# alex-petrenko/sample-factory

Hardware: NVIDIA H100
Metric: env-steps/sec (sampler+learner) at 4096 envs (higher is better)
Workload: dtype f32 (3-pass tf32 hi/lo operand split on wgmma, fp32 accumulate)

## Files before the change

sample_factory_b200/csrc/gemm_tc.cu:

```cuda
#include <cuda.h>

#include <cstdlib>
#include <cudaTypedefs.h>

#include "common.cuh"
#include "gemm.h"
#include "heads_tail.cuh"
#include "tc_ptx.cuh"
#include "wgmma_tile.cuh"

namespace sfb {

constexpr int kProducerRegs = 40;
constexpr int kConsumerRegs = 232;

template <bool A_MN, bool B_MN, bool SPLIT3, bool HEADS, bool F16, bool RES, bool DW16>
__device__ __forceinline__ void gemm_tc_body(const CUtensorMap& tmap_a, const CUtensorMap& tmap_b, float* __restrict__ C,
                                             int64_t ldc, int64_t M, int N, int K, int k_chunk, int splits,
                                             const TcEpilogue& epi, const float* __restrict__ a_bound,
                                             const float* __restrict__ b_bound, unsigned long long* __restrict__ trace) {
    static_assert(!F16 || (!A_MN && SPLIT3), "fp16-split engine: K-major activations, 3-pass");
    static_assert(!DW16 || (A_MN && B_MN && SPLIT3 && !HEADS && !F16 && !RES), "fp16 dW form: MN-major operands, plain epilogue");
    if (trace && threadIdx.x == 0) trace[blockIdx.x * kTraceWords + 8] = tc_now();
    using S = TcSmem<F16, DW16>;
    constexpr int KBK = S::KBK;
    constexpr int SA = S::A_STAGES, SB = S::B_STAGES;
    extern __shared__ uint8_t smem_raw[];
    uint8_t* smem = smem_align_1024(smem_raw);
    uint8_t* conv = smem + S::CONV_OFF;
    uint64_t* bars = reinterpret_cast<uint64_t*>(smem + S::BARS_OFF);
    uint64_t* full_a = bars;
    uint64_t* empty_a = bars + SA;
    uint64_t* full_b = bars + 2 * SA;
    uint64_t* empty_b = bars + 2 * SA + SB;
    int* s_last = reinterpret_cast<int*>(bars + 2 * (SA + SB));

    const int warp = threadIdx.x >> 5, lane = threadIdx.x & 31;
    const int tiles_n = (N + TBN - 1) / TBN;
    const int tiles_per_z = tiles_n * (int)((M + TBM - 1) / TBM);
    const int items = tiles_per_z * splits;

    if (threadIdx.x == 0) {
        asm volatile("prefetch.tensormap [%0];" ::"l"(&tmap_a) : "memory");
        asm volatile("prefetch.tensormap [%0];" ::"l"(&tmap_b) : "memory");
        for (int s = 0; s < SA; ++s) {
            mbar_init(&full_a[s], 1);
            mbar_init(&empty_a[s], 256);
// ... 29 lines not shown
                } else if (DW16) {
                    for (int b = 0; b < TBM / 32; ++b) tma_load_2d(pa + b * 4096, &tmap_a, &full_a[sa], (int)tc.m0 + 32 * b, k0);
                } else if (A_MN) {
                    tma_load_2d(pa, &tmap_a, &full_a[sa], (int)tc.m0, k0);
                } else {
                    tma_load_2d(pa, &tmap_a, &full_a[sa], k0, (int)tc.m0);
                }
                mbar_wait(&empty_b[sb], ((g / SB) & 1) ^ 1);
                mbar_expect_tx(&full_b[sb], S::B_SLOT);
                uint8_t* pb = smem + S::B_RING + sb * S::B_SLOT;
                if (F16) tma_load_3d(pb, &tmap_b, &full_b[sb], k0, tc.n0, 0);
                else if (B_MN) tma_load_2d(pb, &tmap_b, &full_b[sb], tc.n0, k0);
                else tma_load_2d(pb, &tmap_b, &full_b[sb], k0, tc.n0);
            }
            if (trace) trace[item * kTraceWords + 7] = tc_now();
            g0 += tc.num_kb;
        }
        return;
    }

    setmaxnreg_inc<kConsumerRegs>();
    const int ct = threadIdx.x - 128;
    const int wg = ct >> 7;

    const int a_shift = (F16 || DW16) ? f16_shift_for_bound(a_bound[0]) : 0;
    const float a_scale = pow2f_int(a_shift);
    const int b_shift = DW16 ? f16_shift_for_bound(b_bound[0]) : kF16WShift;
    const float b_scale = pow2f_int(b_shift);
    auto split_stage = [&](int g) {
        const int sa = g % SA, sb = g % SB;
        const uint8_t* pa = smem + sa * S::A_RAW;
        uint8_t* cv = conv + (g & 1) * S::CONV;
        mbar_wait(&full_a[sa], (g / SA) & 1);
        split_tile<A_MN, SPLIT3>(pa, cv, cv + S::A_HALF, ct);
        mbar_wait(&full_b[sb], (g / SB) & 1);
        split_tile<B_MN, SPLIT3>(smem + S::B_RING + sb * S::B_SLOT, cv + 2 * S::A_HALF, cv + 2 * S::A_HALF + S::B_HALF, ct);
        mbar_arrive(&empty_b[sb]);
        mbar_arrive(&empty_a[sa]);
        fence_proxy_async_smem();
    };
    constexpr int KS = KBK / 32;
    using Frags = F16Frags<KS>;
    auto load_frags = [&](int g, int h, Frags& f) {
        const int sa = g % SA;
        const uint8_t* pa = smem + sa * S::A_RAW;
        if (h == 0) mbar_wait(&full_a[sa], (g / SA) & 1);
// ... 94 lines not shown
                        wgmma_m64n128k8_tf32(cross, da_hi + o, db_lo + o, 1);
                        wgmma_m64n128k8_tf32(cross, da_lo + o, db_hi + o, 1);
                    }
                }
                wgmma_commit();
                if (kb + 1 < tc.num_kb) split_stage(g + 1);
                wgmma_wait_all();
                consumer_sync();
            }
        }
        g0 += tc.num_kb;
        if (tr) tr[4] = tc_now();
        if (F16 || DW16) {
            const float out_scale = pow2f_int(-(a_shift + b_shift));
#pragma unroll
            for (int i = 0; i < 64; ++i) acc[i] = __fmul_rn(fmaf(cross[i], 1.f / 2048.f, acc[i]), out_scale);
        } else if (SPLIT3) {
#pragma unroll
            for (int i = 0; i < 64; ++i) acc[i] += cross[i];
        }
        if (tr) tr[10] = tc_now_after(acc[63]);

        const int64_t row_base = tc.m0 + wg * 64 + ((ct >> 5) & 3) * 16 + (lane >> 2);
        if constexpr (HEADS) {
            switch (epi.act) {
                case SFB200_ACT_ELU: heads_tile<SFB200_ACT_ELU>(acc, tc, row_base, lane, C, ldc, M, N, epi, tr); break;
                case SFB200_ACT_RELU: heads_tile<SFB200_ACT_RELU>(acc, tc, row_base, lane, C, ldc, M, N, epi, tr); break;
                case SFB200_ACT_TANH: heads_tile<SFB200_ACT_TANH>(acc, tc, row_base, lane, C, ldc, M, N, epi, tr); break;
                default: heads_tile<SFB200_ACT_NONE>(acc, tc, row_base, lane, C, ldc, M, N, epi, tr); break;
            }
            if (epi.fin_counters) {
                const int mb = (int)(tc.m0 / TBM);
                __threadfence();
                consumer_sync();
                if (ct == 0) *s_last = (atomicAdd(&epi.fin_counters[mb], 1) == tiles_n - 1) ? 1 : 0;
                consumer_sync();
                if (*s_last) {
                    __threadfence();
                    const float pv = epi.fin.pv_scalar ? *epi.fin.pv_scalar : 0.f;
                    const uint64_t offset = epi.fin.offset_host + (epi.fin.offset_dev ? (uint64_t)*epi.fin.offset_dev : 0ull);
                    for (int r = ct >> 5; r < TBM; r += 8) {
                        const int64_t row = tc.m0 + r;
                        if (row < M) heads_finish_row(epi.head_part, 2 * tiles_n, M, row, lane, epi.fin, pv, offset);
                    }
                    if (ct == 0) epi.fin_counters[mb] = 0;
                }
            }
        } else if constexpr (RES) {
            if (tile_is_whole(tc, TBM, C, ldc, M, N, epi.aux, epi.ld_aux))
                store_tile_whole<3, SFB200_ACT_NONE>(acc, tc, row_base, lane, C, ldc, epi, tr);
            else
                store_tile_residual(acc, tc, row_base, lane, C, ldc, M, N, epi);
        } else {
// ... 95 lines not shown
        v = (e && e[0] == '1') ? 1 : 0;
    }
    return v == 1;
}

static thread_local unsigned long long* g_gemm_trace = nullptr;
static thread_local int64_t g_gemm_trace_words = 0;

static bool operand_ok(const float* p, int64_t ld) {
    return ((reinterpret_cast<uintptr_t>(p) & 15u) == 0) && (ld % 4 == 0) && ld > 0;
}

template <bool A_MN, bool B_MN, bool SPLIT3, bool HEADS, bool F16, bool RES, bool DW16>
static auto tc_kernel() {
    if constexpr (DW16) return gemm_dw_f16_kernel;
    else return gemm_wgmma_kernel<A_MN, B_MN, SPLIT3, HEADS, F16, RES>;
}

template <bool A_MN, bool B_MN, bool SPLIT3, bool HEADS = false, bool F16 = false, bool RES = false, bool DW16 = false>
static int launch_tc(const CUtensorMap& ta, const CUtensorMap& tb, float* C, int64_t ldc, int64_t M, int N, int K,
                     int k_chunk, int splits, const TcEpilogue& epi, cudaStream_t st, const float* a_bound = nullptr,
                     const float* b_bound = nullptr) {
    auto kern = tc_kernel<A_MN, B_MN, SPLIT3, HEADS, F16, RES, DW16>();
    constexpr int smem = TcSmem<F16, DW16>::TOTAL;
    static int ctas_per_sm = 0;
    if (!ctas_per_sm) {
        SFB_CUDA_OK(cudaFuncSetAttribute(kern, cudaFuncAttributeMaxDynamicSharedMemorySize, smem));
        SFB_CUDA_OK(cudaOccupancyMaxActiveBlocksPerMultiprocessor(&ctas_per_sm, kern, TC_THREADS, (size_t)smem));
        SFB_CHECK_ARG(ctas_per_sm > 0, "gemm_wgmma_kernel does not fit on this device");
    }
    const int64_t items = ceil_div(N, TBN) * ceil_div(M, TBM) * splits;
    const int64_t resident = (int64_t)ctas_per_sm * sm_count();
    SFB_CHECK_ARG(!g_gemm_trace || items * kTraceWords <= g_gemm_trace_words,
                  "gemm trace buffer too small: %lld work items need %lld words", (long long)items,
                  (long long)(items * kTraceWords));
    const dim3 grid((unsigned)(items < resident ? items : resident));
    if constexpr (DW16)
        SFB_CUDA_OK(launch_pdl(kern, grid, dim3(TC_THREADS), (size_t)smem, st, ta, tb, C, ldc, M, N, K, k_chunk, splits, epi,
                               a_bound, g_gemm_trace, b_bound));
    else
        SFB_CUDA_OK(launch_pdl(kern, grid, dim3(TC_THREADS), (size_t)smem, st, ta, tb, C, ldc, M, N, K, k_chunk, splits, epi,
                               a_bound, g_gemm_trace));
    SFB_LAUNCH_OK();
    return 0;
}

static int split_k_chunk(int K, int* splits) {
// ... 154 lines not shown
```

sample_factory_b200/csrc/rollout_fused.cu:

```cuda
#include <cuda.h>

#include <cstdlib>

#include "common.cuh"
#include "gemm.h"
#include "heads_tail.cuh"
#include "step_tail.cuh"
#include "tc_ptx.cuh"
#include "wgmma_tile.cuh"

namespace sfb {

constexpr int RF_THREADS = 384;
constexpr int RF_HEAD_AP = 9;
constexpr int RF_MAX_DIM = 128;
constexpr int RF_TRACE_WORDS = 32;
constexpr int RF_PRODUCER_REGS = 40;
constexpr int RF_CONSUMER_REGS = 232;

__host__ __device__ __forceinline__ bool rf_wide(int H2) { return H2 >= 256; }
__host__ __device__ __forceinline__ int rf_bm(int H2) { return rf_wide(H2) ? 64 : 128; }
__host__ __device__ __forceinline__ int rf_bn(int H2) { return rf_wide(H2) ? 256 : 128; }

template <bool F16>
struct RfSmem {
    static constexpr int STAGES = 2;
    static constexpr int KBK = F16 ? 64 : TBK;
    __host__ __device__ static constexpr int slot(int bm, int bn) { return F16 ? (bm + bn) * 256 : (bm + 3 * bn) * 128; }
    __host__ __device__ static constexpr int a_bytes(int bm) { return bm * KBK * 4; }
    __host__ __device__ static constexpr int b_hi(int bm, int bn) { return F16 ? bm * 256 : (bm + bn) * 128; }
    __host__ __device__ static constexpr int stage_tx(int bm, int bn) { return (bm + bn) * KBK * 4; }
    static constexpr int OFF_CONV_END = STAGES * slot(64, 256) + 64 * 256;
    static constexpr int OFF_PART = OFF_CONV_END + (F16 ? 64 * 256 : 0);
    static constexpr int OFF_B1 = OFF_PART + (F16 ? 256 * kHeadPartPad * 4 : 0);
    static constexpr int OFF_B2 = OFF_B1 + (F16 ? 256 * 4 : 0);
    static constexpr int OFF_HW = OFF_B2 + (F16 ? 256 * 4 : 0);
    static constexpr int OFF_HB = OFF_HW + (F16 ? RF_HEAD_AP * 256 * 4 : 0);
    static constexpr int OFF_BARS = OFF_HB + (F16 ? 16 * 4 : 0);
    static constexpr int OFF_CSTAT = OFF_BARS + 64;
    static constexpr int TOTAL = OFF_CSTAT + 2 * RF_MAX_DIM * 4 + 1024 ;
    static_assert(2 * STAGES * 8 <= 64 && TOTAL + 64 <= 227 * 1024, "shared memory");
    static_assert(STAGES * slot(128, 128) + 128 * 256 <= OFF_PART, "the 128 x 128 layout fits below the partials");
    static_assert(a_bytes(64) % 1024 == 0 && slot(64, 256) % 1024 == 0 && OFF_CONV_END % 1024 == 0,
                  "h1 staging boxes (slot A regions, conversion buffer, the buffer after it) on 1024 B swizzle atoms");
};


struct RolloutArgs {
    int64_t N; int T, K1, H1, H2;
    const float* b1; const float* b2; const float* wv; const float* wa; int A; const float* bv; const float* ba;
    float* h1; float* part; float* x_norm;
    float* values; int64_t values_rs; float* logits; int64_t logits_rs; float* actions; int64_t actions_rs;
    int32_t* env_actions; float* log_prob; int64_t lp_rs; float* pv_out; int64_t pv_rs; const float* pv_scalar;
    const float* noise; uint64_t seed; int64_t* sampler_step;
    const float* tape; int64_t tape_len; int64_t env_off; int term_period, trunc_period; int64_t* env_step;
    float* env_obs; float* env_rew; uint8_t* env_term; uint8_t* env_trunc;
    EpisodeArgs e;
    float* traj_obs; int64_t traj_obs_rs; const float* rnn; int rnn_dim; float* traj_rnn; int64_t traj_rnn_rs;
    ObsNorm n;
    unsigned long long* trace;
    const float* bound_x; const float* bound_h1;
};

__device__ __forceinline__ void cluster_arrive() { asm volatile("barrier.cluster.arrive.release.aligned;" ::: "memory"); }
__device__ __forceinline__ void cluster_wait() { asm volatile("barrier.cluster.wait.acquire.aligned;" ::: "memory"); }
__device__ __forceinline__ void cluster_sync_all() {
    cluster_arrive();
    cluster_wait();
}
__device__ __forceinline__ void fence_proxy_async_all() { asm volatile("fence.proxy.async.global;" ::: "memory"); }
__device__ __forceinline__ unsigned long long rf_now() {
    unsigned long long t;
    asm volatile("mov.u64 %0, %%globaltimer;" : "=l"(t));
    return t;
}
__device__ __forceinline__ uint32_t smid() {
    uint32_t r;
    asm volatile("mov.u32 %0, %%smid;" : "=r"(r));
    return r;
}
__device__ __forceinline__ uint32_t mapa_shared(uint32_t addr, uint32_t rank) {
    uint32_t r;
    asm volatile("mapa.shared::cluster.u32 %0, %1, %2;" : "=r"(r) : "r"(addr), "r"(rank));
    return r;
}
__device__ __forceinline__ void st_cluster_f4(uint32_t addr, float4 v) {
    asm volatile("st.shared::cluster.v4.f32 [%0], {%1, %2, %3, %4};" ::"r"(addr), "f"(v.x), "f"(v.y), "f"(v.z), "f"(v.w)
                 : "memory");
}
__device__ __forceinline__ uint32_t cluster_ctarank() {
    uint32_t r;
    asm volatile("mov.u32 %0, %%cluster_ctarank;" : "=r"(r));
    return r;
}

template <bool F16>
__device__ __forceinline__ void rf_produce(const CUtensorMap* tmap_x, const CUtensorMap* tmap_w1, const CUtensorMap* tmap_h1,
                                           const CUtensorMap* tmap_w2, int T, int K1, int H1, int bm, int bn, int m0, int n0,
                                           uint8_t* smem, uint64_t* full, uint64_t* empty, bool leader) {
    using S = RfSmem<F16>;
    constexpr int KBK = S::KBK;
    const int slot_bytes = S::slot(bm, bn), b_off = S::a_bytes(bm);
    const uint32_t stage_tx = (uint32_t)S::stage_tx(bm, bn);
    const int n1 = K1 / KBK, n2 = H1 / KBK;
    uint32_t pu = 0;
    auto weight = [&](const CUtensorMap* tb, int kb) {
        const uint32_t s = pu % S::STAGES;
        mbar_wait(&empty[s], ((pu / S::STAGES) & 1) ^ 1);
        mbar_expect_tx(&full[s], stage_tx);
        uint8_t* dst = smem + s * slot_bytes + b_off;
        if (F16) tma_load_3d(dst, tb, &full[s], 64 * kb, n0, 0);
// ... 140 lines not shown
#pragma unroll
        for (int jj = 0; jj < 16; ++jj) {
            const int j = 16 * h + jj;
            const int r = rt + 8 * (j & 1), c = (j >> 1) & 7;
            const float v0 = act_fwd_fast(acc[2 * j] + b[j & ~1], act);
            const float v1 = act_fwd_fast(acc[2 * j + 1] + b[j | 1], act);
            uint32_t hv, lv;
            f16_split2(v0 * scale, v1 * scale, hv, lv);
            uint8_t* dst = box[h] + r * 128 + (((c ^ r) & 7) << 4) + 4 * (lane & 3);
            *reinterpret_cast<uint32_t*>(dst) = hv;
            *reinterpret_cast<uint32_t*>(dst + plane_bytes) = lv;
        }
        fence_proxy_async_smem();
        consumer_sync();
        if (issuer) {
            tma_store_3d(tmap_h1, box[h], n0 + 64 * h, m0, 0);
            bulk_commit();
        }
    }
}

template <int ACT>
__device__ __forceinline__ void rf_heads_tile(float (&acc)[64], int nl, int p0, int rb, int lane, const float* b2,
                                              const float* hw, int A, uint32_t part, int rpc) {
    constexpr int JP = 16;
    const int nq = nl + 2 * (lane & 3);
    float b[32];
#pragma unroll
    for (int c = 0; c < 16; ++c) {
        b[2 * c] = b2[nq + 8 * c];
        b[2 * c + 1] = b2[nq + 8 * c + 1];
    }
#pragma unroll
    for (int j = 0; j < 32; ++j) {
        acc[2 * j] = act_fwd_ct<ACT>(acc[2 * j] + b[j & ~1]);
        acc[2 * j + 1] = act_fwd_ct<ACT>(acc[2 * j + 1] + b[j | 1]);
    }
#pragma unroll
    for (int half = 0; half < 2; ++half) {
        float hp[2][kHeadAP];
#pragma unroll
        for (int a = 0; a < kHeadAP; ++a) {
            float s[2] = {0.f, 0.f};
            if (a <= A) {
                const float* w = hw + a * 256 + nq + 64 * half;
                float2 wv[JP / 2];
#pragma unroll
                for (int jj = 0; jj < JP / 2; ++jj) wv[jj] = *reinterpret_cast<const float2*>(w + 8 * jj);
#pragma unroll
                for (int jj = 0; jj < JP / 2; ++jj) {
#pragma unroll
                    for (int rs = 0; rs < 2; ++rs) {
                        const int j = JP * half + 2 * jj + rs;
                        s[rs] = fmaf(acc[2 * j], wv[jj].x, s[rs]);
                        s[rs] = fmaf(acc[2 * j + 1], wv[jj].y, s[rs]);
                    }
                }
            }
#pragma unroll
            for (int rs = 0; rs < 2; ++rs) {
                s[rs] += __shfl_xor_sync(0xffffffffu, s[rs], 1);
                s[rs] += __shfl_xor_sync(0xffffffffu, s[rs], 2);
                hp[rs][a] = s[rs];
            }
        }
        if ((lane & 3) == 0) {
#pragma unroll
            for (int rs = 0; rs < 2; ++rs) {
                const int r = rb + 8 * rs;
                const uint32_t dst =
                    mapa_shared(part + (uint32_t)(((p0 + half) * rpc + r % rpc) * kHeadPartPad * 4), (uint32_t)(r / rpc));
                st_cluster_f4(dst, make_float4(hp[rs][0], hp[rs][1], hp[rs][2], hp[rs][3]));
                st_cluster_f4(dst + 16, make_float4(hp[rs][4], hp[rs][5], hp[rs][6], hp[rs][7]));
                st_cluster_f4(dst + 32, make_float4(hp[rs][8], 0.f, 0.f, 0.f));
            }
        }
    }
}

template <int ACT, bool F16>
__global__ void __launch_bounds__(RF_THREADS, 1)
rollout_mlp2_tape_kernel(const __grid_constant__ CUtensorMap tmap_x, const __grid_constant__ CUtensorMap tmap_w1,
                         const __grid_constant__ CUtensorMap tmap_h1, const __grid_constant__ CUtensorMap tmap_w2,
                         const RolloutArgs a) {
    using S = RfSmem<F16>;
    constexpr int KBK = S::KBK;
    extern __shared__ uint8_t smem_raw[];
    uint8_t* smem = smem_align_1024(smem_raw);
    uint64_t* full = reinterpret_cast<uint64_t*>(smem + S::OFF_BARS);
    uint64_t* empty = full + S::STAGES;
    float* cstat = reinterpret_cast<float*>(smem + S::OFF_CSTAT);
    float* s_part = reinterpret_cast<float*>(smem + S::OFF_PART);
    float* s_b1 = reinterpret_cast<float*>(smem + S::OFF_B1);
    float* s_b2 = reinterpret_cast<float*>(smem + S::OFF_B2);
    float* s_hw = reinterpret_cast<float*>(smem + S::OFF_HW);
    float* s_hb = reinterpret_cast<float*>(smem + S::OFF_HB);

    __shared__ double s_stats[5];
    const int warp = threadIdx.x >> 5, lane = threadIdx.x & 31;
    if (threadIdx.x < 5) s_stats[threadIdx.x] = 0.0;
    const int cx = (int)cluster_ctarank();
    const int CX = gridDim.x;
    const bool wide = rf_wide(a.H2);
    const int BM = rf_bm(a.H2), BN = rf_bn(a.H2);
    const int n0 = cx * BN;
    const int64_t m0 = (int64_t)blockIdx.y * BM;
    const int P = a.H2 / 64;
    const bool do_rms = a.n.mean != nullptr;
    unsigned long long* cta_trace =
        a.trace ? a.trace + (int64_t)a.T * RF_TRACE_WORDS + 4 * ((int64_t)blockIdx.y * gridDim.x + blockIdx.x) : nullptr;
    if (cta_trace && threadIdx.x == 0) {
        cta_trace[0] = smid();
        cta_trace[1] = rf_now();
    }

    if (threadIdx.x == 0) {
        asm volatile("prefetch.tensormap [%0];" ::"l"(&tmap_x) : "memory");
        asm volatile("prefetch.tensormap [%0];" ::"l"(&tmap_w1) : "memory");
        asm volatile("prefetch.tensormap [%0];" ::"l"(&tmap_h1) : "memory");
        asm volatile("prefetch.tensormap [%0];" ::"l"(&tmap_w2) : "memory");
        for (int s = 0; s < S::STAGES; ++s) {
            mbar_init(&full[s], 1);
            mbar_init(&empty[s], 256);
        }
        fence_barrier_init();
    }
    __syncthreads();
    pdl_wait();
    pdl_trigger();
    if (cta_trace && threadIdx.x == 0) cta_trace[2] = rf_now();
    if (do_rms) fill_col_stats(a.n, a.K1, cstat);
    if (F16) {
        for (int i = threadIdx.x; i < BN; i += RF_THREADS) {
            s_b1[i] = a.b1[n0 + i];
            s_b2[i] = a.b2[n0 + i];
            s_hw[i] = a.wv[n0 + i];
            for (int r = 0; r < a.A; ++r) s_hw[(r + 1) * 256 + i] = a.wa[(int64_t)r * a.H2 + n0 + i];
        }
        if (threadIdx.x <= a.A) s_hb[threadIdx.x] = threadIdx.x == 0 ? a.bv[0] : a.ba[threadIdx.x - 1];
    }
    __syncthreads();
    const int64_t env_step0 = a.env_step[0];
    const uint64_t philox0 = a.sampler_step ? (uint64_t)*a.sampler_step : 0ull;

    if (warp < 4) {
        setmaxnreg_dec<RF_PRODUCER_REGS>();
        rf_produce<F16>(&tmap_x, &tmap_w1, &tmap_h1, &tmap_w2, a.T, a.K1, a.H1, BM, BN, (int)m0, n0, smem, full, empty,
                        threadIdx.x == 0);
    } else {
        setmaxnreg_inc<RF_CONSUMER_REGS>();
        const float pv = a.pv_scalar ? *a.pv_scalar : 0.f;
        const int shift_x = F16 ? f16_shift_for_bound(a.bound_x[0]) : 0;
        const int shift_h = F16 ? f16_shift_for_bound(a.bound_h1[0]) : 0;
        const bool tracer = a.trace != nullptr && blockIdx.x == 0 && blockIdx.y == 0 && threadIdx.x == 128;
#define RF_TRACE(slot) do { if (tracer) a.trace[(int64_t)t * RF_TRACE_WORDS + (slot)] = rf_now(); } while (0)
        uint32_t cu = 0;
        const TcEpilogue epi_heads{1, ACT, a.b2, nullptr, 0, a.wv, a.wa, a.A, a.part};
        const TcEpilogue epi_h1{1, ACT, a.b1, nullptr, 0};
        const int ct = threadIdx.x - 128;
        const int64_t row_base = m0 + (wide ? 0 : (ct >> 7) * 64) + ((ct >> 5) & 3) * 16 + (lane >> 2);
        TileCoord tc;
// ... 8 lines not shown
            RF_TRACE(0);
            unsigned long long* const tr = tracer ? a.trace + (int64_t)t * RF_TRACE_WORDS : nullptr;
            {
                float acc[64], cross[64];
                rf_tile<F16, true>(a.K1 / KBK, wide, smem, full, empty, cu, acc, cross, ct, shift_x, tr, 1, 2, 5, -1);
                if (F16) {
                    store_h1_tma(acc, &tmap_h1, tc.n0, (int)m0, (int)(row_base - m0), lane, h1_box, BM * 128, h1_issuer,
                                 s_b1 + (tc.n0 - n0), ACT, pow2f_int(shift_h));
                    RF_TRACE(6);
                    if (h1_issuer) bulk_wait_all();
                } else {
                    store_tile(acc, tc, row_base, lane, a.h1, a.H1, a.N, a.H1, 1, epi_h1);
                    RF_TRACE(6);
                    fence_proxy_async_all();
                }
                RF_TRACE(3);
            }
            cluster_sync_all();
            RF_TRACE(4);
            {
                float acc[64], cross[64];
                rf_tile<F16, !F16>(a.H1 / KBK, wide, smem, full, empty, cu, acc, cross, ct, shift_h, tr, 11, 14, 12, 16);
                if (F16)
                    rf_heads_tile<ACT>(acc, tc.n0 - n0, tc.n0 / 64, (int)(row_base - m0), lane, s_b2, s_hw, a.A,
                                       smem_u32(s_part), BM / CX);
                else
                    heads_tile<ACT>(acc, tc, row_base, lane, nullptr, 0, a.N, a.H2, epi_heads);
                RF_TRACE(7);
            }
            cluster_sync_all();
            RF_TRACE(8);

            {
                const int g = lane & 7;
                const int grp = lane >> 3;
                const int act_idx = (g + 7) & 7;
                const bool has_logit = act_idx < a.A;
                const bool leader = g == 0;
                const bool last = (t + 1 == a.T);
                const int64_t step = env_step0 + t;
                const uint64_t offset = philox0 + (uint64_t)t;
                const float* src_step = a.tape + ((step + 1) % a.tape_len) * a.N * a.K1;
                const float* noise_t = a.noise ? a.noise + (int64_t)t * a.N * a.A : nullptr;
                const int rpc = BM / CX;
                for (int base = 0; base < rpc; base += 32) {
                    const int rr = base + (warp - 4) * 4 + grp;
                    const int64_t row = m0 + cx * rpc + rr;
// ... 291 lines not shown
```

sample_factory_b200/csrc/tc_ptx.cuh:

```cuda
#pragma once
#include <cuda.h>
#include <cudaTypedefs.h>

#include "common.cuh"

namespace sfb {

constexpr int TBM = 128;
constexpr int TBN = 128;
constexpr int TBK = 32;
constexpr int WG_K = 8;

__device__ __forceinline__ uint32_t smem_u32(const void* p) { return (uint32_t)__cvta_generic_to_shared(p); }
__device__ __forceinline__ uint8_t* smem_align_1024(uint8_t* raw) {
    return raw + ((1024u - (smem_u32(raw) & 1023u)) & 1023u);
}

__device__ __forceinline__ void mbar_init(uint64_t* bar, uint32_t count) {
    asm volatile("mbarrier.init.shared::cta.b64 [%0], %1;" ::"r"(smem_u32(bar)), "r"(count));
}
__device__ __forceinline__ void mbar_expect_tx(uint64_t* bar, uint32_t bytes) {
    asm volatile("mbarrier.arrive.expect_tx.shared::cta.b64 _, [%0], %1;" ::"r"(smem_u32(bar)), "r"(bytes) : "memory");
}
__device__ __forceinline__ void mbar_arrive(uint64_t* bar) {
// ... 94 lines not shown
}

__device__ __forceinline__ void wgmma_m64n128k16_f16(float (&d)[64], uint64_t desc_a, uint64_t desc_b, uint32_t scale_d) {
    asm volatile(
        "{\n"
        ".reg .pred p;\n"
        "setp.ne.b32 p, %66, 0;\n"
        "wgmma.mma_async.sync.aligned.m64n128k16.f32.f16.f16 "
        "{%0,%1,%2,%3,%4,%5,%6,%7,%8,%9,%10,%11,%12,%13,%14,%15,%16,%17,%18,%19,%20,%21,%22,%23,%24,%25,%26,%27,%28,%29,%30,%31,%32,%33,%34,%35,%36,%37,%38,%39,%40,%41,%42,%43,%44,%45,%46,%47,%48,%49,%50,%51,%52,%53,%54,%55,%56,%57,%58,%59,%60,%61,%62,%63}, "
        "%64, %65, p, 1, 1, 0, 0;\n"
        "}\n"
        : "+f"(d[0]), "+f"(d[1]), "+f"(d[2]), "+f"(d[3]), "+f"(d[4]), "+f"(d[5]), "+f"(d[6]), "+f"(d[7]), "+f"(d[8]),
          "+f"(d[9]), "+f"(d[10]), "+f"(d[11]), "+f"(d[12]), "+f"(d[13]), "+f"(d[14]), "+f"(d[15]), "+f"(d[16]), "+f"(d[17]),
          "+f"(d[18]), "+f"(d[19]), "+f"(d[20]), "+f"(d[21]), "+f"(d[22]), "+f"(d[23]), "+f"(d[24]), "+f"(d[25]), "+f"(d[26]),
          "+f"(d[27]), "+f"(d[28]), "+f"(d[29]), "+f"(d[30]), "+f"(d[31]), "+f"(d[32]), "+f"(d[33]), "+f"(d[34]), "+f"(d[35]),
          "+f"(d[36]), "+f"(d[37]), "+f"(d[38]), "+f"(d[39]), "+f"(d[40]), "+f"(d[41]), "+f"(d[42]), "+f"(d[43]), "+f"(d[44]),
          "+f"(d[45]), "+f"(d[46]), "+f"(d[47]), "+f"(d[48]), "+f"(d[49]), "+f"(d[50]), "+f"(d[51]), "+f"(d[52]), "+f"(d[53]),
          "+f"(d[54]), "+f"(d[55]), "+f"(d[56]), "+f"(d[57]), "+f"(d[58]), "+f"(d[59]), "+f"(d[60]), "+f"(d[61]), "+f"(d[62]),
          "+f"(d[63])
        : "l"(desc_a), "l"(desc_b), "r"(scale_d));
}

template <int TRANS_B>
__device__ __forceinline__ void wgmma_m64n128k16_f16_rs(float (&d)[64], const uint32_t (&a)[4], uint64_t desc_b) {
    asm volatile(
        "{\n"
        ".reg .pred p;\n"
        "setp.ne.b32 p, %70, 0;\n"
        "wgmma.mma_async.sync.aligned.m64n128k16.f32.f16.f16 "
        "{%0,%1,%2,%3,%4,%5,%6,%7,%8,%9,%10,%11,%12,%13,%14,%15,%16,%17,%18,%19,%20,%21,%22,%23,%24,%25,%26,%27,%28,%29,%30,%31,%32,%33,%34,%35,%36,%37,%38,%39,%40,%41,%42,%43,%44,%45,%46,%47,%48,%49,%50,%51,%52,%53,%54,%55,%56,%57,%58,%59,%60,%61,%62,%63}, "
        "{%64, %65, %66, %67}, %68, p, 1, 1, %69;\n"
        "}\n"
        : "+f"(d[0]), "+f"(d[1]), "+f"(d[2]), "+f"(d[3]), "+f"(d[4]), "+f"(d[5]), "+f"(d[6]), "+f"(d[7]), "+f"(d[8]),
          "+f"(d[9]), "+f"(d[10]), "+f"(d[11]), "+f"(d[12]), "+f"(d[13]), "+f"(d[14]), "+f"(d[15]), "+f"(d[16]), "+f"(d[17]),
          "+f"(d[18]), "+f"(d[19]), "+f"(d[20]), "+f"(d[21]), "+f"(d[22]), "+f"(d[23]), "+f"(d[24]), "+f"(d[25]), "+f"(d[26]),
          "+f"(d[27]), "+f"(d[28]), "+f"(d[29]), "+f"(d[30]), "+f"(d[31]), "+f"(d[32]), "+f"(d[33]), "+f"(d[34]), "+f"(d[35]),
          "+f"(d[36]), "+f"(d[37]), "+f"(d[38]), "+f"(d[39]), "+f"(d[40]), "+f"(d[41]), "+f"(d[42]), "+f"(d[43]), "+f"(d[44]),
          "+f"(d[45]), "+f"(d[46]), "+f"(d[47]), "+f"(d[48]), "+f"(d[49]), "+f"(d[50]), "+f"(d[51]), "+f"(d[52]), "+f"(d[53]),
          "+f"(d[54]), "+f"(d[55]), "+f"(d[56]), "+f"(d[57]), "+f"(d[58]), "+f"(d[59]), "+f"(d[60]), "+f"(d[61]), "+f"(d[62]),
          "+f"(d[63])
        : "r"(a[0]), "r"(a[1]), "r"(a[2]), "r"(a[3]), "l"(desc_b), "n"(TRANS_B), "r"(1u));
}

__device__ __forceinline__ uint64_t make_smem_desc(uint32_t smem_addr) {
    uint64_t d = 0;
    d |= (uint64_t)((smem_addr >> 4) & 0x3fff);
    d |= (uint64_t)1 << 16;
    d |= (uint64_t)(1024u >> 4) << 32;
    d |= (uint64_t)1 << 62;
    return d;
}
__device__ __forceinline__ uint64_t make_smem_desc_mn(uint32_t smem_addr) {
    uint64_t d = 0;
    d |= (uint64_t)((smem_addr >> 4) & 0x3fff);
    d |= (uint64_t)(4096u >> 4) << 16;
    d |= (uint64_t)(1024u >> 4) << 32;
    d |= (uint64_t)1 << 62;
    return d;
}
__device__ __forceinline__ uint32_t sw128_offset(int row, int k) {
    return (uint32_t)(row * 128 + ((((k >> 2) ^ row) & 7) << 4) + (k & 3) * 4);
}

template <int ACT>
__device__ __forceinline__ float act_fwd_ct(float z) {
    if (ACT == SFB200_ACT_ELU) {
        float e;
        asm("ex2.approx.ftz.f32 %0, %1;" : "=f"(e) : "f"(z * 1.4426950216293334961f));
        return z > 0.f ? z : e - 1.f;
    }
    if (ACT == SFB200_ACT_RELU) return fmaxf(z, 0.f);
    if (ACT == SFB200_ACT_TANH) return tanhf(z);
    return z;
}
template <int ACT>
__device__ __forceinline__ float act_bwd_ct(float h) {
    if (ACT == SFB200_ACT_ELU) return h > 0.f ? 1.f : h + 1.f;
    if (ACT == SFB200_ACT_RELU) return h > 0.f ? 1.f : 0.f;
// ... 12 lines not shown
```

sample_factory_b200/csrc/wgmma_tile.cuh:

```cuda
#pragma once
#include "common.cuh"
#include "heads_tail.cuh"
#include "tc_ptx.cuh"

namespace sfb {

struct TcEpilogue {
    int mode;
    int act;
    const float* bias;
    const float* aux;
    int64_t ld_aux;
    const float* head_wv;
    const float* head_wa;
    int head_A;
    float* head_part;
    int* fin_counters;
    HeadsFinish fin;
};

constexpr int kHeadAP = 9;
constexpr int kHeadPad = 12;
constexpr int TC_THREADS = 384;

template <bool F16, bool DW16 = false>
struct TcSmem {
    static constexpr int KBK = F16 ? 64 : TBK;
    static constexpr int A_STAGES = F16 ? 3 : DW16 ? 4 : 3;
    static constexpr int B_STAGES = (F16 || DW16) ? 4 : 3;
    static constexpr int A_RAW = TBM * KBK * 4;
    static constexpr int B_SLOT = F16 ? 2 * TBN * 64 * 2 : TBN * TBK * 4;
    static constexpr int A_HALF = TBM * 128;
    static constexpr int B_HALF = DW16 ? TBN * TBK * 2 : TBN * 128;
    static constexpr int CONV = F16 ? 0 : DW16 ? 2 * B_HALF : 2 * A_HALF + 2 * B_HALF;
    static constexpr int CONV_BUFS = F16 ? 0 : DW16 ? 3 : 2;
    static constexpr int B_RING = A_STAGES * A_RAW;
    static constexpr int CONV_OFF = B_RING + B_STAGES * B_SLOT;
    static constexpr int BARS_OFF = CONV_OFF + CONV_BUFS * CONV;
    static constexpr int BARS = 2 * (A_STAGES + B_STAGES) * 8 + 16;
    static constexpr int TOTAL = 1024  + BARS_OFF + BARS;
    static_assert(TOTAL <= 227 * 1024, "shared memory");
};

__device__ __forceinline__ float act_fwd_fast(float z, int act) {
    if (act == SFB200_ACT_ELU) return z > 0.f ? z : (__expf(z) - 1.f);
    return act_fwd(z, act);
}

__device__ __forceinline__ void consumer_sync() { asm volatile("bar.sync 1, 256;" ::: "memory"); }

template <bool MN, bool SPLIT3, int ROWS = TBM, int THREADS = 2 * ROWS>
__device__ __forceinline__ void split_tile(const uint8_t* raw, uint8_t* hi, uint8_t* lo, int ct) {
    static_assert(!MN || (ROWS == TBM && THREADS == 2 * TBM), "MN-major tiles: whole tiles only");
#pragma unroll
    for (int q = 0; q < (ROWS * TBK / 4) / THREADS; ++q) {
        const int i = ct + THREADS * q;
        const float4 v = reinterpret_cast<const float4*>(raw)[i];
        const float e[4] = {v.x, v.y, v.z, v.w};
        if (!MN) {
            const int r = i >> 3, c = i & 7;
            const uint32_t off = (uint32_t)(r * 128 + (((c ^ r) & 7) << 4));
// ... 194 lines not shown
    switch (epi.act) {
        case SFB200_ACT_ELU: store_tile_whole<MODE, SFB200_ACT_ELU>(acc, tc, row_base, lane, C, ldc, epi, tr); break;
        case SFB200_ACT_RELU: store_tile_whole<MODE, SFB200_ACT_RELU>(acc, tc, row_base, lane, C, ldc, epi, tr); break;
        case SFB200_ACT_TANH: store_tile_whole<MODE, SFB200_ACT_TANH>(acc, tc, row_base, lane, C, ldc, epi, tr); break;
        default: store_tile_whole<MODE, SFB200_ACT_NONE>(acc, tc, row_base, lane, C, ldc, epi, tr); break;
    }
}

__device__ __forceinline__ void store_tile_residual(const float (&acc)[64], const TileCoord& tc, int64_t row_base, int lane,
                                                    float* C, int64_t ldc, int64_t M, int N, const TcEpilogue& epi) {
#pragma unroll
    for (int j = 0; j < 32; ++j) {
        const int64_t m = row_base + 8 * (j & 1);
        const int n = tc.n0 + 8 * (j >> 1) + 2 * (lane & 3);
        if (m >= M || n >= N) continue;
        const float* r = epi.aux + m * epi.ld_aux + n;
        float* dst = C + m * ldc + n;
        dst[0] = (acc[2 * j] + epi.bias[n]) + r[0];
        if (n + 1 < N) dst[1] = (acc[2 * j + 1] + epi.bias[n + 1]) + r[1];
    }
}

template <int ACT>
__device__ __forceinline__ void heads_tile(float (&acc)[64], const TileCoord& tc, int64_t row_base, int lane, float* C,
                                           int64_t ldc, int64_t M, int N, const TcEpilogue& epi,
                                           unsigned long long* tr = nullptr) {
    constexpr int JP = 16;
    const int nq = tc.n0 + 2 * (lane & 3);
    float b[32];
    load_bias_pairs(epi.bias, tc.n0, lane, b);
    if (tr) tr[11] = tc_now_after(b[31]);
#pragma unroll
    for (int j = 0; j < 32; ++j) {
        acc[2 * j] = act_fwd_ct<ACT>(acc[2 * j] + b[j & ~1]);
        acc[2 * j + 1] = act_fwd_ct<ACT>(acc[2 * j + 1] + b[j | 1]);
        const int64_t m = row_base + 8 * (j & 1);
        if (C && m < M) *reinterpret_cast<float2*>(C + m * ldc + nq + 8 * (j >> 1)) = make_float2(acc[2 * j], acc[2 * j + 1]);
    }
    if (tr) tr[12] = tc_now_after(acc[63]);
    const int p0 = (tc.n0 / TBN) * 2;
#pragma unroll
    for (int half = 0; half < 2; ++half) {
        float hp[2][kHeadAP];
#pragma unroll
        for (int a = 0; a < kHeadAP; ++a) {
            float s[2] = {0.f, 0.f};
            if (a <= epi.head_A) {
                const float* w = (a == 0 ? epi.head_wv : epi.head_wa + (int64_t)(a - 1) * N) + nq + 64 * half;
                float2 wv[JP / 2];
#pragma unroll
                for (int jj = 0; jj < JP / 2; ++jj) wv[jj] = __ldg(reinterpret_cast<const float2*>(w + 8 * jj));
#pragma unroll
                for (int jj = 0; jj < JP / 2; ++jj) {
#pragma unroll
                    for (int rs = 0; rs < 2; ++rs) {
                        const int j = JP * half + 2 * jj + rs;
                        s[rs] = fmaf(acc[2 * j], wv[jj].x, s[rs]);
                        s[rs] = fmaf(acc[2 * j + 1], wv[jj].y, s[rs]);
                    }
                }
            }
#pragma unroll
            for (int rs = 0; rs < 2; ++rs) {
                s[rs] += __shfl_xor_sync(0xffffffffu, s[rs], 1);
                s[rs] += __shfl_xor_sync(0xffffffffu, s[rs], 2);
                hp[rs][a] = s[rs];
            }
        }
#pragma unroll
        for (int rs = 0; rs < 2; ++rs) {
            const int64_t m = row_base + 8 * rs;
            if ((lane & 3) == 0 && m < M) {
                float4* dst = reinterpret_cast<float4*>(epi.head_part + ((int64_t)(p0 + half) * M + m) * kHeadPad);
                dst[0] = make_float4(hp[rs][0], hp[rs][1], hp[rs][2], hp[rs][3]);
                dst[1] = make_float4(hp[rs][4], hp[rs][5], hp[rs][6], hp[rs][7]);
                dst[2] = make_float4(hp[rs][8], 0.f, 0.f, 0.f);
            }
        }
    }
    if (tr) tr[13] = tc_now();
}

}
```

Baseline: 36.46 million.

## Compute policy/value head partials with fp16-split wgmma from swizzled smem weights

Replaces the scalar FMA plus shuffle-reduction head projection in the fused heads epilogue (both the standalone TC GEMM and the rollout kernel) with a small fp16 hi/lo split wgmma against head weights pre-packed into swizzled shared memory. It adds per-row dynamic scaling, a new m64n64k16 wgmma wrapper, and a head-weight smem region, which forces the A ring down to two stages for the fp16 heads kernel. The rollout kernel's producer/consumer register split is also shifted toward consumers. This trades CUDA-core FMAs and shuffles for tensor-core work, at the cost of less pipelining depth and fp16-split precision in the head outputs.

```diff
diff --git a/sample_factory_b200/csrc/gemm_tc.cu b/sample_factory_b200/csrc/gemm_tc.cu
--- a/sample_factory_b200/csrc/gemm_tc.cu
+++ b/sample_factory_b200/csrc/gemm_tc.cu
@@ -22,7 +22,7 @@
     static_assert(!F16 || (!A_MN && SPLIT3), "fp16-split engine: K-major activations, 3-pass");
     static_assert(!DW16 || (A_MN && B_MN && SPLIT3 && !HEADS && !F16 && !RES), "fp16 dW form: MN-major operands, plain epilogue");
     if (trace && threadIdx.x == 0) trace[blockIdx.x * kTraceWords + 8] = tc_now();
-    using S = TcSmem<F16, DW16>;
+    using S = TcSmem<F16, DW16, HEADS>;
     constexpr int KBK = S::KBK;
     constexpr int SA = S::A_STAGES, SB = S::B_STAGES;
     extern __shared__ uint8_t smem_raw[];
@@ -98,6 +98,11 @@
     setmaxnreg_inc<kConsumerRegs>();
     const int ct = threadIdx.x - 128;
     const int wg = ct >> 7;
+    if constexpr (HEADS && F16) {
+        fill_head_weights_f16(smem + S::HW_OFF, epi.head_wv, epi.head_wa, epi.head_A, N, 0, N, ct, 256);
+        fence_proxy_async_smem();
+        consumer_sync();
+    }
 
     const int a_shift = (F16 || DW16) ? f16_shift_for_bound(a_bound[0]) : 0;
     const float a_scale = pow2f_int(a_shift);
@@ -238,13 +243,23 @@
         if (tr) tr[10] = tc_now_after(acc[63]);
 
         const int64_t row_base = tc.m0 + wg * 64 + ((ct >> 5) & 3) * 16 + (lane >> 2);
-        if constexpr (HEADS) {
+        if constexpr (HEADS && F16) {
+            const uint32_t hw = smem_u32(smem + S::HW_OFF);
+            switch (epi.act) {
+                case SFB200_ACT_ELU: heads_tile_f16<SFB200_ACT_ELU>(acc, tc, row_base, lane, C, ldc, M, epi, hw, tr); break;
+                case SFB200_ACT_RELU: heads_tile_f16<SFB200_ACT_RELU>(acc, tc, row_base, lane, C, ldc, M, epi, hw, tr); break;
+                case SFB200_ACT_TANH: heads_tile_f16<SFB200_ACT_TANH>(acc, tc, row_base, lane, C, ldc, M, epi, hw, tr); break;
+                default: heads_tile_f16<SFB200_ACT_NONE>(acc, tc, row_base, lane, C, ldc, M, epi, hw, tr); break;
+            }
+        } else if constexpr (HEADS) {
             switch (epi.act) {
                 case SFB200_ACT_ELU: heads_tile<SFB200_ACT_ELU>(acc, tc, row_base, lane, C, ldc, M, N, epi, tr); break;
                 case SFB200_ACT_RELU: heads_tile<SFB200_ACT_RELU>(acc, tc, row_base, lane, C, ldc, M, N, epi, tr); break;
                 case SFB200_ACT_TANH: heads_tile<SFB200_ACT_TANH>(acc, tc, row_base, lane, C, ldc, M, N, epi, tr); break;
                 default: heads_tile<SFB200_ACT_NONE>(acc, tc, row_base, lane, C, ldc, M, N, epi, tr); break;
             }
+        }
+        if constexpr (HEADS) {
             if (epi.fin_counters) {
                 const int mb = (int)(tc.m0 / TBM);
                 __threadfence();
@@ -386,7 +401,7 @@
                      int k_chunk, int splits, const TcEpilogue& epi, cudaStream_t st, const float* a_bound = nullptr,
                      const float* b_bound = nullptr) {
     auto kern = tc_kernel<A_MN, B_MN, SPLIT3, HEADS, F16, RES, DW16>();
-    constexpr int smem = TcSmem<F16, DW16>::TOTAL;
+    constexpr int smem = TcSmem<F16, DW16, HEADS>::TOTAL;
     static int ctas_per_sm = 0;
     if (!ctas_per_sm) {
         SFB_CUDA_OK(cudaFuncSetAttribute(kern, cudaFuncAttributeMaxDynamicSharedMemorySize, smem));
diff --git a/sample_factory_b200/csrc/rollout_fused.cu b/sample_factory_b200/csrc/rollout_fused.cu
--- a/sample_factory_b200/csrc/rollout_fused.cu
+++ b/sample_factory_b200/csrc/rollout_fused.cu
@@ -15,8 +15,8 @@
 constexpr int RF_HEAD_AP = 9;
 constexpr int RF_MAX_DIM = 128;
 constexpr int RF_TRACE_WORDS = 32;
-constexpr int RF_PRODUCER_REGS = 40;
-constexpr int RF_CONSUMER_REGS = 232;
+constexpr int RF_PRODUCER_REGS = 24;
+constexpr int RF_CONSUMER_REGS = 240;
 
 __host__ __device__ __forceinline__ bool rf_wide(int H2) { return H2 >= 256; }
 __host__ __device__ __forceinline__ int rf_bm(int H2) { return rf_wide(H2) ? 64 : 128; }
@@ -35,7 +35,7 @@
     static constexpr int OFF_B1 = OFF_PART + (F16 ? 256 * kHeadPartPad * 4 : 0);
     static constexpr int OFF_B2 = OFF_B1 + (F16 ? 256 * 4 : 0);
     static constexpr int OFF_HW = OFF_B2 + (F16 ? 256 * 4 : 0);
-    static constexpr int OFF_HB = OFF_HW + (F16 ? RF_HEAD_AP * 256 * 4 : 0);
+    static constexpr int OFF_HB = OFF_HW + (F16 ? (256 / TBN) * kHeadTileBytes : 0);
     static constexpr int OFF_BARS = OFF_HB + (F16 ? 16 * 4 : 0);
     static constexpr int OFF_CSTAT = OFF_BARS + 64;
     static constexpr int TOTAL = OFF_CSTAT + 2 * RF_MAX_DIM * 4 + 1024 ;
@@ -43,6 +43,7 @@
     static_assert(STAGES * slot(128, 128) + 128 * 256 <= OFF_PART, "the 128 x 128 layout fits below the partials");
     static_assert(a_bytes(64) % 1024 == 0 && slot(64, 256) % 1024 == 0 && OFF_CONV_END % 1024 == 0,
                   "h1 staging boxes (slot A regions, conversion buffer, the buffer after it) on 1024 B swizzle atoms");
+    static_assert(OFF_HW % 1024 == 0, "the head operand on 1024 B swizzle atoms");
 };
 
 
@@ -84,9 +85,8 @@
     asm volatile("mapa.shared::cluster.u32 %0, %1, %2;" : "=r"(r) : "r"(addr), "r"(rank));
     return r;
 }
-__device__ __forceinline__ void st_cluster_f4(uint32_t addr, float4 v) {
-    asm volatile("st.shared::cluster.v4.f32 [%0], {%1, %2, %3, %4};" ::"r"(addr), "f"(v.x), "f"(v.y), "f"(v.z), "f"(v.w)
-                 : "memory");
+__device__ __forceinline__ void st_cluster_f2(uint32_t addr, float2 v) {
+    asm volatile("st.shared::cluster.v2.f32 [%0], {%1, %2};" ::"r"(addr), "f"(v.x), "f"(v.y) : "memory");
 }
 __device__ __forceinline__ uint32_t cluster_ctarank() {
     uint32_t r;
@@ -273,9 +273,8 @@
 
 template <int ACT>
 __device__ __forceinline__ void rf_heads_tile(float (&acc)[64], int nl, int p0, int rb, int lane, const float* b2,
-                                              const float* hw, int A, uint32_t part, int rpc) {
-    constexpr int JP = 16;
-    const int nq = nl + 2 * (lane & 3);
+                                              uint32_t hw, uint32_t part, int rpc) {
+    const int q = lane & 3, nq = nl + 2 * q;
     float b[32];
 #pragma unroll
     for (int c = 0; c < 16; ++c) {
@@ -287,46 +286,18 @@
         acc[2 * j] = act_fwd_ct<ACT>(acc[2 * j] + b[j & ~1]);
         acc[2 * j + 1] = act_fwd_ct<ACT>(acc[2 * j + 1] + b[j | 1]);
     }
-#pragma unroll
-    for (int half = 0; half < 2; ++half) {
-        float hp[2][kHeadAP];
-#pragma unroll
-        for (int a = 0; a < kHeadAP; ++a) {
-            float s[2] = {0.f, 0.f};
-            if (a <= A) {
-                const float* w = hw + a * 256 + nq + 64 * half;
-                float2 wv[JP / 2];
-#pragma unroll
-                for (int jj = 0; jj < JP / 2; ++jj) wv[jj] = *reinterpret_cast<const float2*>(w + 8 * jj);
-#pragma unroll
-                for (int jj = 0; jj < JP / 2; ++jj) {
-#pragma unroll
-                    for (int rs = 0; rs < 2; ++rs) {
-                        const int j = JP * half + 2 * jj + rs;
-                        s[rs] = fmaf(acc[2 * j], wv[jj].x, s[rs]);
-                        s[rs] = fmaf(acc[2 * j + 1], wv[jj].y, s[rs]);
-                    }
-                }
-            }
-#pragma unroll
-            for (int rs = 0; rs < 2; ++rs) {
-                s[rs] += __shfl_xor_sync(0xffffffffu, s[rs], 1);
-                s[rs] += __shfl_xor_sync(0xffffffffu, s[rs], 2);
-                hp[rs][a] = s[rs];
-            }
-        }
-        if ((lane & 3) == 0) {
-#pragma unroll
-            for (int rs = 0; rs < 2; ++rs) {
-                const int r = rb + 8 * rs;
-                const uint32_t dst =
-                    mapa_shared(part + (uint32_t)(((p0 + half) * rpc + r % rpc) * kHeadPartPad * 4), (uint32_t)(r / rpc));
-                st_cluster_f4(dst, make_float4(hp[rs][0], hp[rs][1], hp[rs][2], hp[rs][3]));
-                st_cluster_f4(dst + 16, make_float4(hp[rs][4], hp[rs][5], hp[rs][6], hp[rs][7]));
-                st_cluster_f4(dst + 32, make_float4(hp[rs][8], 0.f, 0.f, 0.f));
-            }
-        }
-    }
+    float hp[2][8];
+    head_partials_f16<64>(acc, hw + (uint32_t)(nl / TBN) * kHeadTileBytes, hp);
+#pragma unroll
+    for (int half = 0; half < 2; ++half)
+#pragma unroll
+        for (int rs = 0; rs < 2; ++rs) {
+            const int r = rb + 8 * rs;
+            const uint32_t dst = mapa_shared(part + (uint32_t)((((p0 + half) * rpc + r % rpc) * kHeadPartPad + 2 * q) * 4),
+                                             (uint32_t)(r / rpc));
+            st_cluster_f2(dst, make_float2(hp[half][2 * rs], hp[half][2 * rs + 1]));
+            if (q < 2) st_cluster_f2(dst + 32, make_float2(hp[half][4 + 2 * rs], hp[half][5 + 2 * rs]));
+        }
 }
 
 template <int ACT, bool F16>
@@ -344,7 +315,7 @@
     float* s_part = reinterpret_cast<float*>(smem + S::OFF_PART);
     float* s_b1 = reinterpret_cast<float*>(smem + S::OFF_B1);
     float* s_b2 = reinterpret_cast<float*>(smem + S::OFF_B2);
-    float* s_hw = reinterpret_cast<float*>(smem + S::OFF_HW);
+    uint8_t* s_hw = smem + S::OFF_HW;
     float* s_hb = reinterpret_cast<float*>(smem + S::OFF_HB);
 
     __shared__ double s_stats[5];
@@ -385,9 +356,9 @@
         for (int i = threadIdx.x; i < BN; i += RF_THREADS) {
             s_b1[i] = a.b1[n0 + i];
             s_b2[i] = a.b2[n0 + i];
-            s_hw[i] = a.wv[n0 + i];
-            for (int r = 0; r < a.A; ++r) s_hw[(r + 1) * 256 + i] = a.wa[(int64_t)r * a.H2 + n0 + i];
-        }
+        }
+        fill_head_weights_f16(s_hw, a.wv, a.wa, a.A, a.H2, n0, BN, threadIdx.x, RF_THREADS);
+        fence_proxy_async_smem();
         if (threadIdx.x <= a.A) s_hb[threadIdx.x] = threadIdx.x == 0 ? a.bv[0] : a.ba[threadIdx.x - 1];
     }
     __syncthreads();
@@ -442,7 +413,7 @@
                 float acc[64], cross[64];
                 rf_tile<F16, !F16>(a.H1 / KBK, wide, smem, full, empty, cu, acc, cross, ct, shift_h, tr, 11, 14, 12, 16);
                 if (F16)
-                    rf_heads_tile<ACT>(acc, tc.n0 - n0, tc.n0 / 64, (int)(row_base - m0), lane, s_b2, s_hw, a.A,
+                    rf_heads_tile<ACT>(acc, tc.n0 - n0, tc.n0 / 64, (int)(row_base - m0), lane, s_b2, smem_u32(s_hw),
                                        smem_u32(s_part), BM / CX);
                 else
                     heads_tile<ACT>(acc, tc, row_base, lane, nullptr, 0, a.N, a.H2, epi_heads);
diff --git a/sample_factory_b200/csrc/tc_ptx.cuh b/sample_factory_b200/csrc/tc_ptx.cuh
--- a/sample_factory_b200/csrc/tc_ptx.cuh
+++ b/sample_factory_b200/csrc/tc_ptx.cuh
@@ -140,7 +140,8 @@
 }
 
 template <int TRANS_B>
-__device__ __forceinline__ void wgmma_m64n128k16_f16_rs(float (&d)[64], const uint32_t (&a)[4], uint64_t desc_b) {
+__device__ __forceinline__ void wgmma_m64n128k16_f16_rs(float (&d)[64], const uint32_t (&a)[4], uint64_t desc_b,
+                                                        uint32_t scale_d = 1) {
     asm volatile(
         "{\n"
         ".reg .pred p;\n"
@@ -157,7 +158,21 @@
           "+f"(d[45]), "+f"(d[46]), "+f"(d[47]), "+f"(d[48]), "+f"(d[49]), "+f"(d[50]), "+f"(d[51]), "+f"(d[52]), "+f"(d[53]),
           "+f"(d[54]), "+f"(d[55]), "+f"(d[56]), "+f"(d[57]), "+f"(d[58]), "+f"(d[59]), "+f"(d[60]), "+f"(d[61]), "+f"(d[62]),
           "+f"(d[63])
-        : "r"(a[0]), "r"(a[1]), "r"(a[2]), "r"(a[3]), "l"(desc_b), "n"(TRANS_B), "r"(1u));
+        : "r"(a[0]), "r"(a[1]), "r"(a[2]), "r"(a[3]), "l"(desc_b), "n"(TRANS_B), "r"(scale_d));
+}
+
+__device__ __forceinline__ void wgmma_m64n64k16_f16_rs_mn(float (&d)[32], const uint32_t (&a)[4], uint64_t desc_b,
+                                                          uint32_t scale_d) {
+    asm volatile(
+        "{\n"
+        ".reg .pred p;\n"
+        "setp.ne.b32 p, %37, 0;\n"
+        "wgmma.mma_async.sync.aligned.m64n64k16.f32.f16.f16 "
+        "{%0,%1,%2,%3,%4,%5,%6,%7,%8,%9,%10,%11,%12,%13,%14,%15,%16,%17,%18,%19,%20,%21,%22,%23,%24,%25,%26,%27,%28,%29,%30,%31}, "
+        "{%32, %33, %34, %35}, %36, p, 1, 1, 1;\n"
+        "}\n"
+        : "+f"(d[0]), "+f"(d[1]), "+f"(d[2]), "+f"(d[3]), "+f"(d[4]), "+f"(d[5]), "+f"(d[6]), "+f"(d[7]), "+f"(d[8]), "+f"(d[9]), "+f"(d[10]), "+f"(d[11]), "+f"(d[12]), "+f"(d[13]), "+f"(d[14]), "+f"(d[15]), "+f"(d[16]), "+f"(d[17]), "+f"(d[18]), "+f"(d[19]), "+f"(d[20]), "+f"(d[21]), "+f"(d[22]), "+f"(d[23]), "+f"(d[24]), "+f"(d[25]), "+f"(d[26]), "+f"(d[27]), "+f"(d[28]), "+f"(d[29]), "+f"(d[30]), "+f"(d[31])
+        : "r"(a[0]), "r"(a[1]), "r"(a[2]), "r"(a[3]), "l"(desc_b), "r"(scale_d));
 }
 
 __device__ __forceinline__ uint64_t make_smem_desc(uint32_t smem_addr) {
@@ -168,10 +183,10 @@
     d |= (uint64_t)1 << 62;
     return d;
 }
-__device__ __forceinline__ uint64_t make_smem_desc_mn(uint32_t smem_addr) {
+__device__ __forceinline__ uint64_t make_smem_desc_mn(uint32_t smem_addr, uint32_t lbo = 4096) {
     uint64_t d = 0;
     d |= (uint64_t)((smem_addr >> 4) & 0x3fff);
-    d |= (uint64_t)(4096u >> 4) << 16;
+    d |= (uint64_t)(lbo >> 4) << 16;
     d |= (uint64_t)(1024u >> 4) << 32;
     d |= (uint64_t)1 << 62;
     return d;
diff --git a/sample_factory_b200/csrc/wgmma_tile.cuh b/sample_factory_b200/csrc/wgmma_tile.cuh
--- a/sample_factory_b200/csrc/wgmma_tile.cuh
+++ b/sample_factory_b200/csrc/wgmma_tile.cuh
@@ -22,11 +22,12 @@
 constexpr int kHeadAP = 9;
 constexpr int kHeadPad = 12;
 constexpr int TC_THREADS = 384;
-
-template <bool F16, bool DW16 = false>
+constexpr int kHeadTileBytes = 8192;
+
+template <bool F16, bool DW16 = false, bool HEADS = false>
 struct TcSmem {
     static constexpr int KBK = F16 ? 64 : TBK;
-    static constexpr int A_STAGES = F16 ? 3 : DW16 ? 4 : 3;
+    static constexpr int A_STAGES = (F16 && HEADS) ? 2 : F16 ? 3 : DW16 ? 4 : 3;
     static constexpr int B_STAGES = (F16 || DW16) ? 4 : 3;
     static constexpr int A_RAW = TBM * KBK * 4;
     static constexpr int B_SLOT = F16 ? 2 * TBN * 64 * 2 : TBN * TBK * 4;
@@ -36,7 +37,8 @@
     static constexpr int CONV_BUFS = F16 ? 0 : DW16 ? 3 : 2;
     static constexpr int B_RING = A_STAGES * A_RAW;
     static constexpr int CONV_OFF = B_RING + B_STAGES * B_SLOT;
-    static constexpr int BARS_OFF = CONV_OFF + CONV_BUFS * CONV;
+    static constexpr int HW_OFF = CONV_OFF + CONV_BUFS * CONV;
+    static constexpr int BARS_OFF = HW_OFF + ((F16 && HEADS) ? (512 / TBN) * kHeadTileBytes : 0);
     static constexpr int BARS = 2 * (A_STAGES + B_STAGES) * 8 + 16;
     static constexpr int TOTAL = 1024  + BARS_OFF + BARS;
     static_assert(TOTAL <= 227 * 1024, "shared memory");
@@ -277,22 +279,29 @@
 }
 
 template <int ACT>
+__device__ __forceinline__ void heads_act_tile(float (&acc)[64], const TileCoord& tc, int64_t row_base, int lane, float* C,
+                                               int64_t ldc, int64_t M, const TcEpilogue& epi, unsigned long long* tr) {
+    const int nq = tc.n0 + 2 * (lane & 3);
+    float b[32];
+    load_bias_pairs(epi.bias, tc.n0, lane, b);
+    if (tr) tr[11] = tc_now_after(b[31]);
+#pragma unroll
+    for (int j = 0; j < 32; ++j) {
+        acc[2 * j] = act_fwd_ct<ACT>(acc[2 * j] + b[j & ~1]);
+        acc[2 * j + 1] = act_fwd_ct<ACT>(acc[2 * j + 1] + b[j | 1]);
+        const int64_t m = row_base + 8 * (j & 1);
+        if (C && m < M) *reinterpret_cast<float2*>(C + m * ldc + nq + 8 * (j >> 1)) = make_float2(acc[2 * j], acc[2 * j + 1]);
+    }
+    if (tr) tr[12] = tc_now_after(acc[63]);
+}
+
+template <int ACT>
 __device__ __forceinline__ void heads_tile(float (&acc)[64], const TileCoord& tc, int64_t row_base, int lane, float* C,
                                            int64_t ldc, int64_t M, int N, const TcEpilogue& epi,
                                            unsigned long long* tr = nullptr) {
     constexpr int JP = 16;
     const int nq = tc.n0 + 2 * (lane & 3);
-    float b[32];
-    load_bias_pairs(epi.bias, tc.n0, lane, b);
-    if (tr) tr[11] = tc_now_after(b[31]);
-#pragma unroll
-    for (int j = 0; j < 32; ++j) {
-        acc[2 * j] = act_fwd_ct<ACT>(acc[2 * j] + b[j & ~1]);
-        acc[2 * j + 1] = act_fwd_ct<ACT>(acc[2 * j + 1] + b[j | 1]);
-        const int64_t m = row_base + 8 * (j & 1);
-        if (C && m < M) *reinterpret_cast<float2*>(C + m * ldc + nq + 8 * (j >> 1)) = make_float2(acc[2 * j], acc[2 * j + 1]);
-    }
-    if (tr) tr[12] = tc_now_after(acc[63]);
+    heads_act_tile<ACT>(acc, tc, row_base, lane, C, ldc, M, epi, tr);
     const int p0 = (tc.n0 / TBN) * 2;
 #pragma unroll
     for (int half = 0; half < 2; ++half) {
@@ -336,4 +345,101 @@
     if (tr) tr[13] = tc_now();
 }
 
-}
+__device__ __forceinline__ void fill_head_weights_f16(uint8_t* dst, const float* wv, const float* wa, int A, int64_t ld_wa,
+                                                      int n_begin, int cols, int t, int nthreads) {
+    for (int n = t; n < cols; n += nthreads) {
+        float w[16];
+#pragma unroll
+        for (int a = 0; a < 16; ++a)
+            w[a] = a == 0 ? wv[n_begin + n] : (a < kHeadAP && a <= A) ? wa[(int64_t)(a - 1) * ld_wa + n_begin + n] : 0.f;
+        const int h = (n >> 6) & 1, kr = n & 7;
+        uint8_t* row = dst + (n >> 7) * kHeadTileBytes + ((n >> 4) & 3) * 2048 + ((n >> 3) & 1) * 1024 + kr * 128;
+#pragma unroll
+        for (int a = 0; a < 16; ++a) {
+            uint16_t hi, lo;
+            f16_split1(w[a] * (float)(1 << kF16WShift), hi, lo);
+            const int nh = 32 * h + a, nl = nh + 16;
+            *reinterpret_cast<uint16_t*>(row + ((((nh >> 3) ^ kr) & 7) << 4) + (nh & 7) * 2) = hi;
+            *reinterpret_cast<uint16_t*>(row + ((((nl >> 3) ^ kr) & 7) << 4) + (nl & 7) * 2) = lo;
+        }
+    }
+}
+
+template <int N>
+__device__ __forceinline__ void head_partials_f16(const float (&y)[64], uint32_t hw, float (&hp)[2][8]) {
+    static_assert(N == 64 || N == 128, "m64n64k16 or m64n128k16");
+    int shift[2][2];
+#pragma unroll
+    for (int h = 0; h < 2; ++h)
+#pragma unroll
+        for (int rs = 0; rs < 2; ++rs) {
+            float mx = 0.f;
+#pragma unroll
+            for (int jj = 0; jj < 8; ++jj) {
+                const int i = 32 * h + 4 * jj + 2 * rs;
+                mx = fmaxf(mx, fmaxf(fabsf(y[i]), fabsf(y[i + 1])));
+            }
+            mx = fmaxf(mx, __shfl_xor_sync(0xffffffffu, mx, 1));
+            mx = fmaxf(mx, __shfl_xor_sync(0xffffffffu, mx, 2));
+            shift[h][rs] = f16_shift_for_bound(mx);
+        }
+#pragma unroll
+    for (int h = 0; h < 2; ++h) {
+        F16Frags<4> f;
+#pragma unroll
+        for (int kk = 0; kk < 4; ++kk)
+#pragma unroll
+            for (int j = 0; j < 4; ++j) {
+                const int i = 32 * h + 8 * kk + 2 * j;
+                const float sc = pow2f_int(shift[h][j & 1]);
+                f16_split2(y[i] * sc, y[i + 1] * sc, f.hi[kk][j], f.lo[kk][j]);
+            }
+#pragma unroll
+        for (int k = 0; k < 4; ++k)
+#pragma unroll
+            for (int j = 0; j < 4; ++j) asm volatile("" : "+r"(f.hi[k][j]), "+r"(f.lo[k][j]));
+        float d[N / 2];
+        float (&part)[8] = hp[h];
+#pragma unroll
+        for (int pass = 0; pass < 2; ++pass) {
+            wgmma_fence();
+#pragma unroll
+            for (int kk = 0; kk < 4; ++kk) {
+                const uint64_t db = make_smem_desc_mn(hw + kk * 2048, 0);
+                if constexpr (N == 128) wgmma_m64n128k16_f16_rs<1>(d, pass ? f.lo[kk] : f.hi[kk], db, kk != 0);
+                else wgmma_m64n64k16_f16_rs_mn(d, pass ? f.lo[kk] : f.hi[kk], db, kk != 0);
+            }
+            wgmma_commit();
+            wgmma_wait_all();
+#pragma unroll
+            for (int i = 0; i < 8; ++i) {
+                if (pass == 0) part[i] = fmaf(d[16 * h + 8 + i], 1.f / 2048.f, d[16 * h + i]);
+                else part[i] = __fmul_rn(fmaf(d[16 * h + i], 1.f / 2048.f, part[i]),
+                                         pow2f_int(-(shift[h][(i >> 1) & 1] + kF16WShift)));
+            }
+        }
+    }
+}
+
+template <int ACT>
+__device__ __forceinline__ void heads_tile_f16(float (&acc)[64], const TileCoord& tc, int64_t row_base, int lane, float* C,
+                                               int64_t ldc, int64_t M, const TcEpilogue& epi, uint32_t hw,
+                                               unsigned long long* tr) {
+    heads_act_tile<ACT>(acc, tc, row_base, lane, C, ldc, M, epi, tr);
+    const int p0 = (tc.n0 / TBN) * 2, q = lane & 3;
+    float hp[2][8];
+    head_partials_f16<128>(acc, hw + (uint32_t)(tc.n0 / TBN) * kHeadTileBytes, hp);
+#pragma unroll
+    for (int half = 0; half < 2; ++half)
+#pragma unroll
+        for (int rs = 0; rs < 2; ++rs) {
+            const int64_t m = row_base + 8 * rs;
+            if (m >= M) continue;
+            float* dst = epi.head_part + ((int64_t)(p0 + half) * M + m) * kHeadPad + 2 * q;
+            *reinterpret_cast<float2*>(dst) = make_float2(hp[half][2 * rs], hp[half][2 * rs + 1]);
+            if (q < 2) *reinterpret_cast<float2*>(dst + 8) = make_float2(hp[half][4 + 2 * rs], hp[half][5 + 2 * rs]);
+        }
+    if (tr) tr[13] = tc_now();
+}
+
+}
```

Measured after the change: 37.71 million (median of 6 runs). 3.4% higher.
